# Luca96/carla-driving-rl-agent

Hardware: AMD Instinct MI355X
Metric: PPO update-steps/sec (batch=256, 4x90x120x3 obs) (higher is better)
Workload: dtype f32; 1 GPU; configs[1]: synthetic rollout buffer 256x4-frame 90x120x3 obs per GPU, full CARLANetwork fwd/bwd + PPO (re-sampled Beta, pathwise) / value loss + clip + Adam, fp32; per_gpu_batch=256, global_batch=256, parallelism=dp1, policy_loss=resampled (reference-faithful)

## Files before the change

### carla-driving-rl-agent_amd/csrc/gemm_tn_lds.hip

```cpp
#include <stdlib.h>

#include "colreduce.h"

namespace cdrl {

typedef float f32x16 __attribute__((ext_vector_type(16)));
typedef __bf16 bf16x8 __attribute__((ext_vector_type(8)));

struct TnLdsArgs {
    View A, D;
    float* part;
    int M, N, K, G, Mg;
    int rows_per, nspg;
    const float* a_stats;
    TnBnBwd db;
};

constexpr int TNL_R = 32;

template <int MODE, bool APRO, bool DPRO>
__global__ void __launch_bounds__(256, 2) tn_lds_kernel(TnLdsArgs a) {
    constexpr bool BH = MODE == 2, F32 = MODE == 0, X3 = MODE == 3;
    constexpr int NBUF = X3 ? 1 : 2, PL = X3 ? 3 : 1;
    constexpr int TNL_CS = F32 ? TNL_R + 1 : TNL_R / 2 + 1;
    __shared__ uint32_t AsT[NBUF * PL][128 * TNL_CS];
    __shared__ uint32_t DsT[NBUF * PL][128 * TNL_CS];
    constexpr uint32_t ESZ = BH ? 2u : 4u;
    const int tid = threadIdx.x, lane = tid & 63, wave = tid >> 6;
    const int l32 = lane & 31, lh = lane >> 5;
    const int K = a.K, N = a.N;
    const int k0 = blockIdx.y * 128, n0 = blockIdx.z * 128;
    const int KT = min(4, (K - k0 + 31) / 32), NT = min(4, (N - n0 + 31) / 32);
    const int grp = blockIdx.x / a.nspg;
    const int64_t gend = (int64_t)(grp + 1) * a.Mg;
    const int64_t mbeg64 = (int64_t)grp * a.Mg + (int64_t)(blockIdx.x % a.nspg) * a.rows_per;
    const int mb = (int)mbeg64;
    const int me = (int)min(mbeg64 + a.rows_per, gend);
    const int rg = tid >> 5, cq = tid & 31;
    const int ka = k0 + 4 * cq, nd = n0 + 4 * cq;
    float asc[4], ash[4], qm[4], qi[4], qsc[4], qsh[4], qk1[4], qk2[4], qk3[4];
#pragma unroll
    for (int j = 0; j < 4; ++j) {
        asc[j] = 1.0f;
        ash[j] = 0.0f;
        if (APRO) {
            const bool on = ka + j < K;
            asc[j] = on ? a.a_stats[2 * a.G * K + grp * K + ka + j] : 0.0f;
            ash[j] = on ? a.a_stats[3 * a.G * K + grp * K + ka + j] : 0.0f;
        }
        qm[j] = qi[j] = qsc[j] = qsh[j] = qk1[j] = qk2[j] = qk3[j] = 0.0f;
        if (DPRO && nd + j < N) {
            const int GN = a.G * N, o = grp * N + nd + j;
            qm[j] = a.db.stats[0 * GN + o];
            qi[j] = a.db.stats[1 * GN + o];
            qsc[j] = a.db.stats[2 * GN + o];
            qsh[j] = a.db.stats[3 * GN + o];
            qk1[j] = a.db.coef[0 * GN + o];
            qk2[j] = a.db.coef[1 * GN + o];
            qk3[j] = a.db.coef[2 * GN + o];
        }
    }
    const bool relu = DPRO && a.db.act == ACT_RELU6;
    const uint32_t OOR = 0x80000000u;
    const __amdgpu_buffer_rsrc_t rA =
        __builtin_amdgcn_make_buffer_rsrc(const_cast<float*>(a.A.p), 0, (int)((int64_t)a.M * a.A.ld * ESZ), 0x00020000);
    const __amdgpu_buffer_rsrc_t rD =
        __builtin_amdgcn_make_buffer_rsrc(const_cast<float*>(a.D.p), 0, (int)((int64_t)a.M * a.D.ld * ESZ), 0x00020000);
    const __amdgpu_buffer_rsrc_t rY = __builtin_amdgcn_make_buffer_rsrc(
        const_cast<float*>(DPRO ? a.db.y : a.D.p), 0, (int)((int64_t)a.M * (DPRO ? N : a.D.ld) * ESZ), 0x00020000);
    const bool a4 = (ka + 3 < K);
    const bool a2 = (ka + 1 < K);
    const bool d4 = (nd + 3 < N), d2 = (nd + 1 < N);
    const int shuf = DPRO ? a.db.shuffle_ctot : 0;
    uint32_t voA = a2 ? (uint32_t)(a.A.coff + ka) * ESZ : OOR;
    uint32_t voD0, voD1;
    const bool dhalf = shuf && d2 && !d4;
    if (shuf) {
        voD0 = d2 ? (uint32_t)(shuffle_dst(a.D.coff + nd, shuf) - (dhalf ? 1 : 0)) * ESZ : OOR;
        voD1 = d2 ? (uint32_t)(shuffle_dst(a.D.coff + nd + 1, shuf) - (dhalf ? 1 : 0)) * ESZ : OOR;
    } else {
        voD0 = d2 ? (uint32_t)(a.D.coff + nd) * ESZ : OOR;
        voD1 = d4 ? (uint32_t)(a.D.coff + nd + 2) * ESZ : OOR;
    }
    const uint32_t voY = d2 ? (uint32_t)nd * ESZ : OOR;
    const uint32_t sA = (uint32_t)a.A.ld * ESZ, sD = (uint32_t)a.D.ld * ESZ, sY = (uint32_t)N * ESZ;
    typedef uint32_t u32x2_t __attribute__((ext_vector_type(2)));
    auto ld2 = [&](const __amdgpu_buffer_rsrc_t& rs, uint32_t vo, uint32_t ro, float& x0, float& x1) {
        const uint32_t off = (vo & 0x80000000u) ? 0x80000000u : vo + ro;
        if (BH) {
            const uint32_t w = __builtin_amdgcn_raw_buffer_load_b32(rs, off, 0, 0);
            x0 = bf_lo(w);
            x1 = bf_hi(w);
        } else {
            const u32x2_t w = __builtin_amdgcn_raw_buffer_load_b64(rs, off, 0, 0);
            x0 = __uint_as_float(w[0]);
            x1 = __uint_as_float(w[1]);
        }
    };
    struct Regs {
        float a[4][4], d[4][4], y[DPRO ? 4 : 1][DPRO ? 4 : 1];
    };
    auto load_chunk = [&](int m0, Regs& r) {
#pragma unroll
        for (int i = 0; i < 4; ++i) {
            const int m = m0 + 4 * rg + i;
            const uint32_t msk = m < me ? 0u : OOR;
            const uint32_t row = (uint32_t)m;
            ld2(rA, voA | msk, row * sA, r.a[i][0], r.a[i][1]);
            ld2(rA, (a4 ? voA + 2 * ESZ : OOR) | msk, row * sA, r.a[i][2], r.a[i][3]);
            if (shuf) {
                ld2(rD, voD0 | msk, row * sD, r.d[i][0], r.d[i][2]);
                ld2(rD, voD1 | msk, row * sD, r.d[i][1], r.d[i][3]);
                if (dhalf) {
                    r.d[i][0] = r.d[i][2];
                    r.d[i][1] = r.d[i][3];
                    r.d[i][2] = r.d[i][3] = 0.0f;
                }
            } else {
                ld2(rD, voD0 | msk, row * sD, r.d[i][0], r.d[i][1]);
                ld2(rD, voD1 | msk, row * sD, r.d[i][2], r.d[i][3]);
            }
            if (DPRO) {
                ld2(rY, voY | msk, row * sY, r.y[DPRO ? i : 0][0], r.y[DPRO ? i : 0][DPRO ? 1 : 0]);
                ld2(rY, (d4 ? voY + 2 * ESZ : OOR) | msk, row * sY, r.y[DPRO ? i : 0][DPRO ? 2 : 0], r.y[DPRO ? i : 0][DPRO ? 3 : 0]);
            }
        }
        __builtin_amdgcn_sched_barrier(0);
    };
    auto store_chunk = [&](int m0, int buf, const Regs& r) {
        float keep[4];
#pragma unroll
        for (int i = 0; i < 4; ++i) keep[i] = (m0 + 4 * rg + i) < me ? 1.0f : 0.0f;
#pragma unroll
        for (int j = 0; j < 4; ++j) {
            float x[4], d[4];
#pragma unroll
            for (int i = 0; i < 4; ++i) {
                x[i] = r.a[i][j];
                if (APRO) x[i] = fmaf(asc[j], x[i], ash[j]);
                d[i] = r.d[i][j];
                if (DPRO) {
                    const float y = r.y[DPRO ? i : 0][DPRO ? j : 0];
                    if (relu) {
                        const float z = fmaf(qsc[j], y, qsh[j]);
                        d[i] = relu6_open(z) ? d[i] : 0.0f;
                    }
                    const float xh = (y - qm[j]) * qi[j];
                    d[i] = keep[i] * (qk1[j] * (d[i] - qk2[j] - xh * qk3[j]));
                }
            }
            const int c = 4 * cq + j;
            if (F32) {
                uint32_t* pa = &AsT[buf][c * TNL_CS + 4 * rg];
                uint32_t* pd = &DsT[buf][c * TNL_CS + 4 * rg];
#pragma unroll
                for (int i = 0; i < 4; ++i) {
                    pa[i] = __float_as_uint(x[i]);
                    pd[i] = __float_as_uint(d[i]);
                }
            } else if (X3) {
#pragma unroll
                for (int pl = 0; pl < 3; ++pl) {
                    float hx[4], hd[4];
#pragma unroll
                    for (int i = 0; i < 4; ++i) {
                        hx[i] = (float)(bf16_t)x[i];
                        hd[i] = (float)(bf16_t)d[i];
                        x[i] -= hx[i];
                        d[i] -= hd[i];
                    }
                    uint32_t* pa = &AsT[pl][c * TNL_CS + 2 * rg];
                    pa[0] = bf_pack(hx[0], hx[1]);
                    pa[1] = bf_pack(hx[2], hx[3]);
                    uint32_t* pd = &DsT[pl][c * TNL_CS + 2 * rg];
                    pd[0] = bf_pack(hd[0], hd[1]);
                    pd[1] = bf_pack(hd[2], hd[3]);
                }
            } else {
                uint32_t* pa = &AsT[buf][c * TNL_CS + 2 * rg];
                pa[0] = bf_pack(x[0], x[1]);
                pa[1] = bf_pack(x[2], x[3]);
                uint32_t* pd = &DsT[buf][c * TNL_CS + 2 * rg];
                pd[0] = bf_pack(d[0], d[1]);
                pd[1] = bf_pack(d[2], d[3]);
            }
        }
    };
    f32x16 acc[4];
#pragma unroll
    for (int j = 0; j < 4; ++j)
#pragma unroll
        for (int q = 0; q < 16; ++q) acc[j][q] = 0.0f;
    auto frag = [&](const uint32_t* base, int col, int s) -> bf16x8 {
        const uint32_t* p = base + col * TNL_CS + 8 * s + 4 * lh;
        typedef uint32_t u32x4_t __attribute__((ext_vector_type(4)));
        u32x4_t w;
        w[0] = p[0];
        w[1] = p[1];
        w[2] = p[2];
        w[3] = p[3];
        return __builtin_bit_cast(bf16x8, w);
    };
    auto mma_chunk = [&](int buf) {
        if (wave >= KT) return;
        if (F32) {
            const uint32_t* pa = &AsT[buf][(wave * 32 + l32) * TNL_CS + lh];
#pragma unroll
            for (int s = 0; s < TNL_R / 2; ++s) {
                const float av = __uint_as_float(pa[2 * s]);
#pragma unroll
                for (int j = 0; j < 4; ++j) {
                    if (j < NT) {
                        const float dv = __uint_as_float(DsT[buf][(j * 32 + l32) * TNL_CS + 2 * s + lh]);
                        acc[j] = __builtin_amdgcn_mfma_f32_32x32x2f32(av, dv, acc[j], 0, 0, 0);
                    }
                }
            }
            return;
        }
        if (X3) {
#pragma unroll
            for (int s = 0; s < TNL_R / 16; ++s) {
                const bf16x8 a1 = frag(AsT[0], wave * 32 + l32, s), a2 = frag(AsT[X3 ? 1 : 0], wave * 32 + l32, s),
                             a3 = frag(AsT[X3 ? 2 : 0], wave * 32 + l32, s);
#pragma unroll
                for (int j = 0; j < 4; ++j) {
                    if (j < NT) {
                        const bf16x8 d1 = frag(DsT[0], j * 32 + l32, s), d2 = frag(DsT[X3 ? 1 : 0], j * 32 + l32, s),
                                     d3 = frag(DsT[X3 ? 2 : 0], j * 32 + l32, s);
                        acc[j] = __builtin_amdgcn_mfma_f32_32x32x16_bf16(a2, d2, acc[j], 0, 0, 0);
                        acc[j] = __builtin_amdgcn_mfma_f32_32x32x16_bf16(a3, d1, acc[j], 0, 0, 0);
                        acc[j] = __builtin_amdgcn_mfma_f32_32x32x16_bf16(a1, d3, acc[j], 0, 0, 0);
                        acc[j] = __builtin_amdgcn_mfma_f32_32x32x16_bf16(a2, d1, acc[j], 0, 0, 0);
                        acc[j] = __builtin_amdgcn_mfma_f32_32x32x16_bf16(a1, d2, acc[j], 0, 0, 0);
                        acc[j] = __builtin_amdgcn_mfma_f32_32x32x16_bf16(a1, d1, acc[j], 0, 0, 0);
                    }
                }
            }
            return;
        }
#pragma unroll
        for (int s = 0; s < TNL_R / 16; ++s) {
            const bf16x8 af = frag(AsT[buf], wave * 32 + l32, s);
#pragma unroll
            for (int j = 0; j < 4; ++j) {
                if (j < NT) {
                    const bf16x8 df = frag(DsT[buf], j * 32 + l32, s);
                    acc[j] = __builtin_amdgcn_mfma_f32_32x32x16_bf16(af, df, acc[j], 0, 0, 0);
                }
            }
        }
    };
    Regs r0;
    int c = 0;
    if (mb < me) load_chunk(mb, r0);
    for (int m0 = mb; m0 < me; m0 += TNL_R, ++c) {
        store_chunk(m0, X3 ? 0 : (c & 1), r0);
        __syncthreads();
        if (m0 + TNL_R < me) load_chunk(m0 + TNL_R, r0);
        mma_chunk(X3 ? 0 : (c & 1));
        if (X3) __syncthreads();
    }
    if (wave >= KT) return;
    float* out = a.part + (int64_t)blockIdx.x * K * N;
#pragma unroll
    for (int j = 0; j < 4; ++j) {
        const int n = n0 + j * 32 + l32;
        if (j >= NT || n >= N) continue;
#pragma unroll
        for (int q = 0; q < 16; ++q) {
            const int kk = k0 + wave * 32 + (q & 3) + 8 * (q >> 2) + 4 * lh;
            if (kk < K) out[(int64_t)kk * N + n] = acc[j][q];
        }
    }
}

struct TnlPlan {
    int gy, gz, nspg, nsplit, rows_per;
};

static TnlPlan tnl_plan(int M, int N, int K, int G) {
    TnlPlan p;
    p.gy = cdiv(K, 128);
    p.gz = cdiv(N, 128);
    const int Mg = M / G;
    static const int wgs = 384;
    int target = wgs / (p.gy * p.gz * G);
    if (target < 1) target = 1;
    int ns = Mg / 128;
    if (ns > target) ns = target;
    if (ns < 1) ns = 1;
    p.rows_per = cdiv(cdiv(Mg, ns), TNL_R) * TNL_R;
    p.nspg = cdiv(Mg, p.rows_per);
    p.nsplit = G * p.nspg;
    return p;
}

int64_t gemm_tn_lds_part_elems(int M, int N, int K, int G) { return (int64_t)tnl_plan(M, N, K, G).nsplit * K * N; }

bool gemm_tn_lds_supported(View A, View D, int N, int K, int shuffle_ctot) {
    if ((A.ld & 1) || (A.coff & 1) || (D.ld & 1) || (D.coff & 1) || (K & 1) || (N & 1)) return false;
    if (shuffle_ctot && ((shuffle_ctot >> 1) & 1)) return false;
    return true;
}

void gemm_tn_lds_plan(TnPlan& p, int M, int N, int K, int G, int shuffle_ctot) {
    const TnlPlan q = tnl_plan(M, N, K, G);
    p.kernel = 2;
    p.NJW = p.WK = p.NSPL = p.RS = p.RS2 = p.U = 0;
    p.gy = q.gy;
    p.gz = q.gz;
    p.nspg = q.nspg;
    p.nsplit = q.nsplit;
    p.rows_per = q.rows_per;
    p.part_slots = q.nsplit;
    p.dhalf = (p.dpro && shuffle_ctot && N % 4 == 2) ? 1 : 0;
}

int gemm_tn_lds(const TnPlan& p, View A, View D, float* Cout, int M, int N, int K, float* part, int accumulate, hipStream_t st, int G,
                const float* pro_stats, const TnBnBwd* dpro) {
    if (!p.ok || p.kernel != 2 || !gemm_tn_lds_supported(A, D, N, K, dpro ? dpro->shuffle_ctot : 0)) {
        set_error("gemm_tn_lds: not planned for this call (K=%d N=%d)", K, N);
        return -1;
    }
    TnLdsArgs a;
    a.A = A;
    a.D = D;
    a.part = part;
    a.M = M;
    a.N = N;
    a.K = K;
    a.G = G;
    a.Mg = M / G;
    a.rows_per = p.rows_per;
    a.nspg = p.nspg;
    a.a_stats = pro_stats;
    a.db = TnBnBwd{};
    if (dpro) a.db = *dpro;
    const dim3 grid(p.nsplit, p.gy, p.gz), blk(256);
    const bool ap = p.apro != 0, dp = p.dpro != 0;
#define CDRL_TNL(BHV)                                                                               \
    do {                                                                                            \
        if (ap && dp) hipLaunchKernelGGL((tn_lds_kernel<BHV, true, true>), grid, blk, 0, st, a);    \
        else if (ap) hipLaunchKernelGGL((tn_lds_kernel<BHV, true, false>), grid, blk, 0, st, a);    \
        else if (dp) hipLaunchKernelGGL((tn_lds_kernel<BHV, false, true>), grid, blk, 0, st, a);    \
        else hipLaunchKernelGGL((tn_lds_kernel<BHV, false, false>), grid, blk, 0, st, a);           \
    } while (0)
    switch (p.mode) {
        case 2: CDRL_TNL(2); break;
        case 3: CDRL_TNL(3); break;
        case 0: CDRL_TNL(0); break;
        default: CDRL_TNL(1); break;
    }
#undef CDRL_TNL
    CDRL_LAUNCH_CHECK();
    const int64_t n = (int64_t)K * N;
    return reduce_partials_f32(part, p.part_slots, n, n, Cout, accumulate, st);
}

}
```

Before: 78.41 update-steps/s.

## Swizzle bf16 LDS tiles for vector access and software-pipeline X3 MFMA fragments

Replaces the padded bf16 LDS layout in the TN gradient GEMM with an XOR-swizzled slot layout. This allows 64-bit stores and 128-bit fragment reads without bank conflicts, and the thread-to-row/column mapping is remapped to match. It adds a software-pipelined X3 (split-bf16 triple) MFMA path that prefetches the next fragments while issuing the current six MFMAs. It also moves the coefficient loads after the first global load and issues the next chunk load before the barrier in X3 mode. The risk is register pressure under launch bounds (256,2) and correctness of the remapped indices.

```diff
diff --git a/carla-driving-rl-agent_amd/csrc/gemm_tn_lds.hip b/carla-driving-rl-agent_amd/csrc/gemm_tn_lds.hip
--- a/carla-driving-rl-agent_amd/csrc/gemm_tn_lds.hip
+++ b/carla-driving-rl-agent_amd/csrc/gemm_tn_lds.hip
@@ -18,13 +18,15 @@
 
 constexpr int TNL_R = 32;
 
+__device__ __forceinline__ int tnl_slot(int c, int q) { return 16 * (32 * (c & 3) + (c >> 2)) + 4 * (q ^ (c & 3) ^ ((c >> 3) & 3)); }
+
 template <int MODE, bool APRO, bool DPRO>
 __global__ void __launch_bounds__(256, 2) tn_lds_kernel(TnLdsArgs a) {
     constexpr bool BH = MODE == 2, F32 = MODE == 0, X3 = MODE == 3;
     constexpr int NBUF = X3 ? 1 : 2, PL = X3 ? 3 : 1;
-    constexpr int TNL_CS = F32 ? TNL_R + 1 : TNL_R / 2 + 1;
-    __shared__ uint32_t AsT[NBUF * PL][128 * TNL_CS];
-    __shared__ uint32_t DsT[NBUF * PL][128 * TNL_CS];
+    constexpr int TNL_CS = F32 ? TNL_R + 1 : TNL_R / 2;
+    __shared__ __attribute__((aligned(16))) uint32_t AsT[NBUF * PL][128 * TNL_CS];
+    __shared__ __attribute__((aligned(16))) uint32_t DsT[NBUF * PL][128 * TNL_CS];
     constexpr uint32_t ESZ = BH ? 2u : 4u;
     const int tid = threadIdx.x, lane = tid & 63, wave = tid >> 6;
     const int l32 = lane & 31, lh = lane >> 5;
@@ -36,30 +38,33 @@
     const int64_t mbeg64 = (int64_t)grp * a.Mg + (int64_t)(blockIdx.x % a.nspg) * a.rows_per;
     const int mb = (int)mbeg64;
     const int me = (int)min(mbeg64 + a.rows_per, gend);
-    const int rg = tid >> 5, cq = tid & 31;
+    const int rg = F32 ? tid >> 5 : 2 * wave + (BH ? lane & 1 : (lane >> 3) & 1);
+    const int cq = F32 ? tid & 31 : BH ? lane >> 1 : (lane & 7) | ((lane >> 4) << 3);
     const int ka = k0 + 4 * cq, nd = n0 + 4 * cq;
     float asc[4], ash[4], qm[4], qi[4], qsc[4], qsh[4], qk1[4], qk2[4], qk3[4];
-#pragma unroll
-    for (int j = 0; j < 4; ++j) {
-        asc[j] = 1.0f;
-        ash[j] = 0.0f;
-        if (APRO) {
-            const bool on = ka + j < K;
-            asc[j] = on ? a.a_stats[2 * a.G * K + grp * K + ka + j] : 0.0f;
-            ash[j] = on ? a.a_stats[3 * a.G * K + grp * K + ka + j] : 0.0f;
-        }
-        qm[j] = qi[j] = qsc[j] = qsh[j] = qk1[j] = qk2[j] = qk3[j] = 0.0f;
-        if (DPRO && nd + j < N) {
-            const int GN = a.G * N, o = grp * N + nd + j;
-            qm[j] = a.db.stats[0 * GN + o];
-            qi[j] = a.db.stats[1 * GN + o];
-            qsc[j] = a.db.stats[2 * GN + o];
-            qsh[j] = a.db.stats[3 * GN + o];
-            qk1[j] = a.db.coef[0 * GN + o];
-            qk2[j] = a.db.coef[1 * GN + o];
-            qk3[j] = a.db.coef[2 * GN + o];
-        }
-    }
+    auto load_coefs = [&]() {
+#pragma unroll
+        for (int j = 0; j < 4; ++j) {
+            asc[j] = 1.0f;
+            ash[j] = 0.0f;
+            if (APRO) {
+                const bool on = ka + j < K;
+                asc[j] = on ? a.a_stats[2 * a.G * K + grp * K + ka + j] : 0.0f;
+                ash[j] = on ? a.a_stats[3 * a.G * K + grp * K + ka + j] : 0.0f;
+            }
+            qm[j] = qi[j] = qsc[j] = qsh[j] = qk1[j] = qk2[j] = qk3[j] = 0.0f;
+            if (DPRO && nd + j < N) {
+                const int GN = a.G * N, o = grp * N + nd + j;
+                qm[j] = a.db.stats[0 * GN + o];
+                qi[j] = a.db.stats[1 * GN + o];
+                qsc[j] = a.db.stats[2 * GN + o];
+                qsh[j] = a.db.stats[3 * GN + o];
+                qk1[j] = a.db.coef[0 * GN + o];
+                qk2[j] = a.db.coef[1 * GN + o];
+                qk3[j] = a.db.coef[2 * GN + o];
+            }
+        }
+    };
     const bool relu = DPRO && a.db.act == ACT_RELU6;
     const uint32_t OOR = 0x80000000u;
     const __amdgpu_buffer_rsrc_t rA =
@@ -127,6 +132,12 @@
         }
         __builtin_amdgcn_sched_barrier(0);
     };
+    auto st2 = [](uint32_t* p, uint32_t w0, uint32_t w1) {
+        u32x2_t w;
+        w[0] = w0;
+        w[1] = w1;
+        *reinterpret_cast<u32x2_t*>(p) = w;
+    };
     auto store_chunk = [&](int m0, int buf, const Regs& r) {
         float keep[4];
 #pragma unroll
@@ -150,6 +161,7 @@
                 }
             }
             const int c = 4 * cq + j;
+            const int so = F32 ? 0 : tnl_slot(c, rg >> 1) + 2 * (rg & 1);
             if (F32) {
                 uint32_t* pa = &AsT[buf][c * TNL_CS + 4 * rg];
                 uint32_t* pd = &DsT[buf][c * TNL_CS + 4 * rg];
@@ -169,20 +181,12 @@
                         x[i] -= hx[i];
                         d[i] -= hd[i];
                     }
-                    uint32_t* pa = &AsT[pl][c * TNL_CS + 2 * rg];
-                    pa[0] = bf_pack(hx[0], hx[1]);
-                    pa[1] = bf_pack(hx[2], hx[3]);
-                    uint32_t* pd = &DsT[pl][c * TNL_CS + 2 * rg];
-                    pd[0] = bf_pack(hd[0], hd[1]);
-                    pd[1] = bf_pack(hd[2], hd[3]);
+                    st2(&AsT[pl][so], bf_pack(hx[0], hx[1]), bf_pack(hx[2], hx[3]));
+                    st2(&DsT[pl][so], bf_pack(hd[0], hd[1]), bf_pack(hd[2], hd[3]));
                 }
             } else {
-                uint32_t* pa = &AsT[buf][c * TNL_CS + 2 * rg];
-                pa[0] = bf_pack(x[0], x[1]);
-                pa[1] = bf_pack(x[2], x[3]);
-                uint32_t* pd = &DsT[buf][c * TNL_CS + 2 * rg];
-                pd[0] = bf_pack(d[0], d[1]);
-                pd[1] = bf_pack(d[2], d[3]);
+                st2(&AsT[buf][so], bf_pack(x[0], x[1]), bf_pack(x[2], x[3]));
+                st2(&DsT[buf][so], bf_pack(d[0], d[1]), bf_pack(d[2], d[3]));
             }
         }
     };
@@ -192,14 +196,8 @@
 #pragma unroll
         for (int q = 0; q < 16; ++q) acc[j][q] = 0.0f;
     auto frag = [&](const uint32_t* base, int col, int s) -> bf16x8 {
-        const uint32_t* p = base + col * TNL_CS + 8 * s + 4 * lh;
         typedef uint32_t u32x4_t __attribute__((ext_vector_type(4)));
-        u32x4_t w;
-        w[0] = p[0];
-        w[1] = p[1];
-        w[2] = p[2];
-        w[3] = p[3];
-        return __builtin_bit_cast(bf16x8, w);
+        return __builtin_bit_cast(bf16x8, *reinterpret_cast<const u32x4_t*>(base + tnl_slot(col, 2 * s + lh)));
     };
     auto mma_chunk = [&](int buf) {
         if (wave >= KT) return;
@@ -214,6 +212,38 @@
                         const float dv = __uint_as_float(DsT[buf][(j * 32 + l32) * TNL_CS + 2 * s + lh]);
                         acc[j] = __builtin_amdgcn_mfma_f32_32x32x2f32(av, dv, acc[j], 0, 0, 0);
                     }
+                }
+            }
+            return;
+        }
+        if (X3 && !(APRO && DPRO) && NT == 4) {
+            const int ca = wave * 32 + l32;
+            bf16x8 af[3], df[3], an[3], dn[3];
+#pragma unroll
+            for (int pl = 0; pl < 3; ++pl) {
+                af[pl] = an[pl] = frag(AsT[X3 ? pl : 0], ca, 0);
+                df[pl] = dn[pl] = frag(DsT[X3 ? pl : 0], l32, 0);
+            }
+#pragma unroll
+            for (int g = 0; g < 8; ++g) {
+                const int j = g & 3, sn = (g + 1) >> 2, jn = (g + 1) & 3;
+                if (g + 1 < 8) {
+#pragma unroll
+                    for (int pl = 0; pl < 3; ++pl) {
+                        dn[pl] = frag(DsT[X3 ? pl : 0], jn * 32 + l32, sn);
+                        if (jn == 0) an[pl] = frag(AsT[X3 ? pl : 0], ca, sn);
+                    }
+                }
+                acc[j] = __builtin_amdgcn_mfma_f32_32x32x16_bf16(af[1], df[1], acc[j], 0, 0, 0);
+                acc[j] = __builtin_amdgcn_mfma_f32_32x32x16_bf16(af[2], df[0], acc[j], 0, 0, 0);
+                acc[j] = __builtin_amdgcn_mfma_f32_32x32x16_bf16(af[0], df[2], acc[j], 0, 0, 0);
+                acc[j] = __builtin_amdgcn_mfma_f32_32x32x16_bf16(af[1], df[0], acc[j], 0, 0, 0);
+                acc[j] = __builtin_amdgcn_mfma_f32_32x32x16_bf16(af[0], df[1], acc[j], 0, 0, 0);
+                acc[j] = __builtin_amdgcn_mfma_f32_32x32x16_bf16(af[0], df[0], acc[j], 0, 0, 0);
+#pragma unroll
+                for (int pl = 0; pl < 3; ++pl) {
+                    df[pl] = dn[pl];
+                    af[pl] = an[pl];
                 }
             }
             return;
@@ -254,10 +284,12 @@
     Regs r0;
     int c = 0;
     if (mb < me) load_chunk(mb, r0);
+    load_coefs();
     for (int m0 = mb; m0 < me; m0 += TNL_R, ++c) {
         store_chunk(m0, X3 ? 0 : (c & 1), r0);
+        if (X3 && m0 + TNL_R < me) load_chunk(m0 + TNL_R, r0);
         __syncthreads();
-        if (m0 + TNL_R < me) load_chunk(m0 + TNL_R, r0);
+        if (!X3 && m0 + TNL_R < me) load_chunk(m0 + TNL_R, r0);
         mma_chunk(X3 ? 0 : (c & 1));
         if (X3) __syncthreads();
     }
```

New measurement: 78.95 update-steps/s (median of 6 runs). Within noise of the previous version (+0.7%).
